# Aedelon/ProteinBERT-PyTorch-Replication

Measured on AMD Instinct MI355X. Metric: sequences/sec (whole node) ProteinBERT pretrain L=512 at 1/2/4/8 MI355X, higher is better.
Workload: dtype bf16; 1 GPU; global_batch=2048, per_gpu_batch=2048, seq_len=512, parallelism=dp1, impl=hip, hip_graph=False

## Files before the change

proteinbert_pytorch_replication_amd/ops/csrc/conv4.hip:

```cpp
#include "mfma.h"

using namespace pbx;
typedef unsigned short bf16_t;

namespace {
constexpr int CH = 128;
constexpr int BM = 128;
constexpr int KS = 9;
constexpr int NI = KS * 8;
constexpr int NPT = BM / 32;


struct FinArgs {
  const bf16_t* dh1;
  const bf16_t* s1;
  const float* st1;
  int T1, BM1;
  const float* sums1;
  int TS1;
  const float* g1;
  float* dgb;
  float eps;
};

template <bool FIN>
__global__ void __launch_bounds__(256, 2) conv_dgrad4_kernel(
    const bf16_t* __restrict__ ds1, const bf16_t* __restrict__ gdn, const bf16_t* __restrict__ gdw,
    const bf16x8* __restrict__ ftn, const bf16x8* __restrict__ ftw, bf16_t* __restrict__ dx,
    bf16_t* __restrict__ dpre_n, bf16_t* __restrict__ dpre_w, int L, int dil, int ilo, int ihi, FinArgs fa) {
  extern __shared__ __attribute__((aligned(16))) unsigned char smem[];
  const int T = (L + BM - 1) / BM;
  int tid0;
  {
    const int n = gridDim.x, orig = blockIdx.x, xcd = orig & 7, qq = n >> 3, rr = n & 7;
    tid0 = (xcd < rr ? xcd * (qq + 1) : rr * (qq + 1) + (xcd - rr) * qq) + (orig >> 3);
  }
  const int b = tid0 / T, t = tid0 - (tid0 / T) * T;
  const int pos0 = t * BM;
  const int half = KS >> 1;
  const int halo_n = half, halo_w = half * dil;
  const int RN = BM + 2 * halo_n;
  unsigned char* an = smem;
  unsigned char* aw = smem + RN * 256;
  const int tid = threadIdx.x, lane = tid & 63, cq = __builtin_amdgcn_readfirstlane(tid >> 6);
  const int r = lane & 31, h = lane >> 5;
  const size_t sbase = (size_t)b * L * CH;
  const ptrdiff_t ibase = ((ptrdiff_t)b * (L + ilo + ihi) + ilo) * CH;
  const __amdgpu_buffer_rsrc_t rn = __builtin_amdgcn_make_buffer_rsrc(
      const_cast<bf16x8*>(ftn + cq * 64), (short)0, (NI * 4 - cq) * 1024, 0x00020000);
  const __amdgpu_buffer_rsrc_t rw = __builtin_amdgcn_make_buffer_rsrc(
      const_cast<bf16x8*>(ftw + cq * 64), (short)0, (NI * 4 - cq) * 1024, 0x00020000);
  auto wfrag = [&](int it) {
    typedef __attribute__((ext_vector_type(4))) unsigned int u32x4;
    const int li = it < NI ? it : it - NI;
    const u32x4 v = __builtin_amdgcn_raw_buffer_load_b128(it < NI ? rn : rw, lane * 16, li * 4096, 0);
    return __builtin_bit_cast(bf16x8, v);
  };
  bf16x8 fr[4];
  fr[0] = wfrag(0);
  fr[1] = wfrag(1);
  fr[2] = wfrag(2);

  uint4 keep[9];
  float csum[8];
  float mean1 = 0.f, rstd1 = 0.f, m1 = 0.f, m2 = 0.f;
  if constexpr (FIN) {
    wave_ln_stats(fa.st1 + (size_t)b * fa.T1 * 2, fa.T1, fa.BM1, L, CH, fa.eps, mean1, rstd1);
    wave_bwd_consts(fa.sums1 + (size_t)b * fa.TS1 * 2, fa.TS1, 1.0f / (float)(L * CH), m1, m2);
#pragma unroll
    for (int e = 0; e < 8; ++e) csum[e] = 0.f;
  }
  auto fin_load = [&](int pos, int c16, uint4& qd, uint4& qs, float4& ga, float4& gb) {
    const int p = min(max(pos, 0), L - 1);
    const size_t off = sbase + (size_t)p * CH + c16 * 8;
    qd = *reinterpret_cast<const uint4*>(fa.dh1 + off);
    qs = *reinterpret_cast<const uint4*>(fa.s1 + off);
    ga = *reinterpret_cast<const float4*>(fa.g1 + (size_t)p * CH + c16 * 8);
    gb = *reinterpret_cast<const float4*>(fa.g1 + (size_t)p * CH + c16 * 8 + 4);
  };
  auto fin_ds1 = [&](bool ok, const uint4& qd, const uint4& qs, const float4& ga, const float4& gb) {
    float dv[8], sv[8], o[8];
    unpack8(qd, dv);
    unpack8(qs, sv);
    const float g[8] = {ga.x, ga.y, ga.z, ga.w, gb.x, gb.y, gb.z, gb.w};
#pragma unroll
    for (int e = 0; e < 8; ++e) o[e] = ok ? rstd1 * (dv[e] * g[e] - m1 - (sv[e] - mean1) * rstd1 * m2) : 0.f;
    return packq8(o);
  };
  auto dpre_of = [&](const uint4& gq, const uint4& pq) {
    float g[8], pv[8], o[8];
    unpack8(gq, g);
    unpack8(pq, pv);
#pragma unroll
    for (int e = 0; e < 8; ++e) o[e] = pv[e] * g[e];
    return packq8(o);
  };
  if constexpr (FIN) {
    const int nchw = (BM + 2 * halo_w) * 16;
    const int joff = halo_w - halo_n;
    for (int base = tid; base < nchw; base += 4 * 256) {
      uint4 qd[4], qs[4], pq[4];
      float4 ga[4], gb[4];
#pragma unroll
      for (int i = 0; i < 4; ++i) {
        const int idx = base + i * 256;
        const int pos = pos0 - halo_w + (idx >> 4);
        fin_load(pos, idx & 15, qd[i], qs[i], ga[i], gb[i]);
        pq[i] = *reinterpret_cast<const uint4*>(gdw + sbase + (size_t)min(max(pos, 0), L - 1) * CH + (idx & 15) * 8);
      }
#pragma unroll
      for (int i = 0; i < 4; ++i) {
        const int idx = base + i * 256;
        if (idx >= nchw) break;
        const int j = idx >> 4, ch = idx & 15;
        const int pos = pos0 - halo_w + j;
        const bool ok = pos >= 0 && pos < L;
        const uint4 dq = fin_ds1(ok, qd[i], qs[i], ga[i], gb[i]);
        const uint4 v = ok ? dpre_of(dq, pq[i]) : make_uint4(0u, 0u, 0u, 0u);
        if (ok && j >= halo_w && j < halo_w + BM)
          *reinterpret_cast<uint4*>(dpre_w + sbase + (size_t)pos * CH + ch * 8) = v;
        *reinterpret_cast<uint4*>(aw + swz256(j, ch)) = v;
        if (j >= joff && j < joff + RN) *reinterpret_cast<uint4*>(an + swz256(j - joff, ch)) = dq;
      }
    }
    __syncthreads();
    const int nch = RN * 16;
#pragma unroll
    for (int mb = 0; mb < 9; mb += 3) {
      uint4 pq[3];
#pragma unroll
      for (int i = 0; i < 3; ++i) {
        const int idx = tid + 256 * (mb + i);
        const int pos = pos0 - halo_n + (idx >> 4);
        pq[i] = *reinterpret_cast<const uint4*>(gdn + sbase + (size_t)min(max(pos, 0), L - 1) * CH + (idx & 15) * 8);
      }
#pragma unroll
      for (int i = 0; i < 3; ++i) {
        const int m = mb + i;
        const int idx = tid + 256 * m;
        const int j = idx >> 4, ch = idx & 15;
        const int pos = pos0 - halo_n + j;
        const bool ok = idx < nch && pos >= 0 && pos < L;
        const uint4 dq = idx < nch ? *reinterpret_cast<const uint4*>(an + swz256(j, ch)) : make_uint4(0u, 0u, 0u, 0u);
        keep[m] = dq;
        if (ok && j >= halo_n && j < halo_n + BM) {
          float t[8];
          unpack8(dq, t);
#pragma unroll
          for (int e = 0; e < 8; ++e) csum[e] += t[e];
        }
        if (idx < nch) {
          const uint4 v = ok ? dpre_of(dq, pq[i]) : make_uint4(0u, 0u, 0u, 0u);
          if (ok && j >= halo_n && j < halo_n + BM)
            *reinterpret_cast<uint4*>(dpre_n + sbase + (size_t)pos * CH + ch * 8) = v;
          *reinterpret_cast<uint4*>(an + swz256(j, ch)) = v;
        }
      }
    }
  }
#pragma unroll 1
  for (int c = 0; c < (FIN ? 0 : 2); ++c) {
    const int halo = c ? halo_w : halo_n;
    const bf16_t* gd = c ? gdw : gdn;
    bf16_t* dpo = c ? dpre_w : dpre_n;
    unsigned char* tile = c ? aw : an;
    const int nch = (BM + 2 * halo) * 16;
    for (int base = tid; base < nch; base += 4 * 256) {
      uint4 gq[4], pq[4];
#pragma unroll
      for (int i = 0; i < 4; ++i) {
        const int idx = base + i * 256;
        const int pos = pos0 - halo + (idx >> 4);
        const bool ok = idx < nch && pos >= -ilo && pos < L + ihi;
        const ptrdiff_t off = ibase + (ptrdiff_t)(ok ? pos : 0) * CH + (idx & 15) * 8;
        gq[i] = ok ? *reinterpret_cast<const uint4*>(ds1 + off) : make_uint4(0u, 0u, 0u, 0u);
        pq[i] = ok ? *reinterpret_cast<const uint4*>(gd + off) : make_uint4(0u, 0u, 0u, 0u);
      }
#pragma unroll
      for (int i = 0; i < 4; ++i) {
        const int idx = base + i * 256;
        if (idx >= nch) break;
        const int j = idx >> 4, ch = idx & 15;
        const int pos = pos0 - halo + j;
        float g[8], pv[8], o[8];
        unpack8(gq[i], g);
        unpack8(pq[i], pv);
#pragma unroll
        for (int e = 0; e < 8; ++e) o[e] = pv[e] * g[e];
        const uint4 v = (pos >= -ilo && pos < L + ihi) ? packq8(o) : make_uint4(0u, 0u, 0u, 0u);
        if (pos >= 0 && pos < L && j >= halo && j < halo + BM)
          *reinterpret_cast<uint4*>(dpo + sbase + (size_t)pos * CH + ch * 8) = v;
        *reinterpret_cast<uint4*>(tile + swz256(j, ch)) = v;
      }
    }
  }
  __syncthreads();

  f32x16_t acc[NPT];
#pragma unroll
  for (int i = 0; i < NPT; ++i) acc[i] = zero16();
  auto rows_of = [&](int c, int k, int& rowb, int& gs) {
    const int rb = (c ? halo_w : halo_n) + r - (k - half) * (c ? dil : 1);
    rowb = rb << 8;
    gs = (h ^ (((rb & 3) << 2) | ((rb >> 2) & 3))) << 4;
  };
  bf16x8 bq[2][NPT];
  int rowb, gs;
  rows_of(0, 0, rowb, gs);
#pragma unroll
  for (int pt = 0; pt < NPT; ++pt) bq[0][pt] = lds_frag(an, (0 ^ gs) + rowb + pt * 8192);
#pragma unroll 1
  for (int c = 0; c < 2; ++c) {
    const unsigned char* as = c ? aw : an;
    for (int k = 0; k < KS; ++k) {
      const int cn = k + 1 < KS ? c : 1, kn = k + 1 < KS ? k + 1 : 0;
      const unsigned char* asn = cn ? aw : an;
      int rowbn, gsn;
      rows_of(cn, kn, rowbn, gsn);
#pragma unroll
      for (int kb = 0; kb < 8; ++kb) {
        const int it = c * NI + k * 8 + kb;
        fr[(kb + 3) & 3] = wfrag(min(it + 3, 2 * NI - 1));
        const unsigned char* nb = kb < 7 ? as : asn;
        const int noff = kb < 7 ? ((32 * (kb + 1)) ^ gs) + rowb : (0 ^ gsn) + rowbn;
#pragma unroll
        for (int pt = 0; pt < NPT; ++pt) bq[(kb + 1) & 1][pt] = lds_frag(nb, noff + pt * 8192);
        __builtin_amdgcn_sched_barrier(0);
#pragma unroll
        for (int pt = 0; pt < NPT; ++pt) acc[pt] = mfma32(fr[kb & 3], bq[kb & 1][pt], acc[pt]);
      }
      rowb = rowbn;
      gs = gsn;
    }
  }

  const int vrows = min(BM, L - pos0);
  float* ft = reinterpret_cast<float*>(smem);
  auto fidx = [&](int p, int c4) { return p * CH + ((c4 ^ (p & 31)) << 2); };
  __syncthreads();
#pragma unroll
  for (int pt = 0; pt < NPT; ++pt)
#pragma unroll
    for (int g = 0; g < 4; ++g) {
      const int c4 = (cq * 32 + 8 * g + 4 * h) >> 2;
      *reinterpret_cast<float4*>(ft + fidx(pt * 32 + r, c4)) =
          make_float4(acc[pt][4 * g], acc[pt][4 * g + 1], acc[pt][4 * g + 2], acc[pt][4 * g + 3]);
    }
  if constexpr (FIN) {
#pragma unroll
    for (int e = 0; e < 8; ++e) {
      csum[e] += __shfl_xor(csum[e], 16, 64);
      csum[e] += __shfl_xor(csum[e], 32, 64);
    }
    float* dsum = ft + BM * CH;
    if (lane < 16) {
#pragma unroll
      for (int e = 0; e < 8; ++e) dsum[cq * CH + lane * 8 + e] = csum[e];
    }
  }
  __syncthreads();
  if constexpr (FIN) {
    if (tid < CH) {
      const float* dsum = ft + BM * CH;
      atomicAdd(fa.dgb + (size_t)b * CH + tid, dsum[tid] + dsum[CH + tid] + dsum[2 * CH + tid] + dsum[3 * CH + tid]);
    }
#pragma unroll
    for (int m = 0; m < 9; ++m) {
      const int row = (tid >> 4) + 16 * m - halo_n, cc = tid & 15;
      if (row < 0 || row >= vrows) continue;
      float gv[8], o[8];
      unpack8(keep[m], gv);
      const float4 f0 = *reinterpret_cast<const float4*>(ft + fidx(row, 2 * cc));
      const float4 f1 = *reinterpret_cast<const float4*>(ft + fidx(row, 2 * cc + 1));
      const float fv[8] = {f0.x, f0.y, f0.z, f0.w, f1.x, f1.y, f1.z, f1.w};
#pragma unroll
      for (int e = 0; e < 8; ++e) o[e] = gv[e] + fv[e];
      *reinterpret_cast<uint4*>(dx + sbase + (size_t)(pos0 + row) * CH + cc * 8) = packq8(o);
    }
    return;
  }
#pragma unroll
  for (int i = 0; i < BM * 16 / 256; ++i) {
    const int idx = tid + 256 * i;
    const int row = idx >> 4, cc = idx & 15;
    if (row >= vrows) continue;
    const size_t off = sbase + (size_t)(pos0 + row) * CH + cc * 8;
    float gv[8], o[8];
    unpack8(*reinterpret_cast<const uint4*>(ds1 + ibase + (ptrdiff_t)(pos0 + row) * CH + cc * 8), gv);
    const float4 f0 = *reinterpret_cast<const float4*>(ft + fidx(row, 2 * cc));
    const float4 f1 = *reinterpret_cast<const float4*>(ft + fidx(row, 2 * cc + 1));
    const float fv[8] = {f0.x, f0.y, f0.z, f0.w, f1.x, f1.y, f1.z, f1.w};
#pragma unroll
    for (int e = 0; e < 8; ++e) o[e] = gv[e] + fv[e];
    *reinterpret_cast<uint4*>(dx + off) = packq8(o);
  }
}

bool dgrad4_attr_set = false;
}

int conv_dgrad4_lds(int dil) {
  const int a = (2 * BM + 8 * (1 + dil)) * 256;
  const int e = BM * CH * 4 + 4 * CH * 4;
  return a > e ? a : e;
}

PBX_EXPORT int pbx_conv_dgrad4x(const void* ds1, const void* gdn, const void* gdw, const void* ftn, const void* ftw,
                                void* dx, void* dpre_n, void* dpre_w, int B, int L, int KS_, int dil, int ilo, int ihi,
                                hipStream_t st) {
  const int lds = conv_dgrad4_lds(dil);
  if (KS_ != KS || dil < 1 || lds > 163840 || B < 1 || L < 1 || ilo < 0 || ihi < 0) return (int)hipErrorInvalidValue;
  if (!dgrad4_attr_set) {
    (void)hipFuncSetAttribute((const void*)conv_dgrad4_kernel<false>, hipFuncAttributeMaxDynamicSharedMemorySize, 163840);
    (void)hipFuncSetAttribute((const void*)conv_dgrad4_kernel<true>, hipFuncAttributeMaxDynamicSharedMemorySize, 163840);
    dgrad4_attr_set = true;
  }
  const int T = (L + BM - 1) / BM;
  hipLaunchKernelGGL(conv_dgrad4_kernel<false>, dim3(B * T), dim3(256), lds, st, (const bf16_t*)ds1,
                     (const bf16_t*)gdn, (const bf16_t*)gdw, (const bf16x8*)ftn, (const bf16x8*)ftw, (bf16_t*)dx,
                     (bf16_t*)dpre_n, (bf16_t*)dpre_w, L, dil, ilo, ihi, FinArgs{});
  return pbx_launch_status();
}

PBX_EXPORT int pbx_conv_dgrad4f(const void* dh1, const void* s1, const float* st1, int T1, int BM1, const float* sums1,
                                int TS1, const float* g1, const void* gdn, const void* gdw, const void* ftn,
                                const void* ftw, void* dx, void* dpre_n, void* dpre_w, float* dgb, int B, int L,
                                int KS_, int dil, float eps, hipStream_t st) {
  const int lds = conv_dgrad4_lds(dil);
  if (KS_ != KS || dil < 1 || lds > 163840 || B < 1 || L < 1 || T1 < 1 || BM1 < 1 || TS1 < 1)
    return (int)hipErrorInvalidValue;
  if (!dgrad4_attr_set) {
    (void)hipFuncSetAttribute((const void*)conv_dgrad4_kernel<false>, hipFuncAttributeMaxDynamicSharedMemorySize, 163840);
    (void)hipFuncSetAttribute((const void*)conv_dgrad4_kernel<true>, hipFuncAttributeMaxDynamicSharedMemorySize, 163840);
    dgrad4_attr_set = true;
  }
  const int T = (L + BM - 1) / BM;
  FinArgs fa{(const bf16_t*)dh1, (const bf16_t*)s1, st1, T1, BM1, sums1, TS1, g1, dgb, eps};
  hipLaunchKernelGGL(conv_dgrad4_kernel<true>, dim3(B * T), dim3(256), lds, st, nullptr, (const bf16_t*)gdn,
                     (const bf16_t*)gdw, (const bf16x8*)ftn, (const bf16x8*)ftw, (bf16_t*)dx, (bf16_t*)dpre_n,
                     (bf16_t*)dpre_w, L, dil, 0, 0, fa);
  return pbx_launch_status();
}
```

proteinbert_pytorch_replication_amd/ops/csrc/mfma.h:

```cpp
#pragma once
#include "common.h"

typedef __attribute__((ext_vector_type(8))) __bf16 bf16x8;
typedef __attribute__((ext_vector_type(4))) short s16x4;

namespace pbx {

__device__ __forceinline__ f32x16_t mfma32(const bf16x8& a, const bf16x8& b, const f32x16_t& c) {
  return __builtin_amdgcn_mfma_f32_32x32x16_bf16(a, b, c, 0, 0, 0);
}

__device__ __forceinline__ f32x16_t zero16() {
  f32x16_t z;
#pragma unroll
  for (int i = 0; i < 16; ++i) z[i] = 0.f;
  return z;
}

__device__ __forceinline__ int swz256(int row, int chunk) {
  return (row << 8) + ((chunk ^ (((row & 3) << 2) | ((row >> 2) & 3))) << 4);
}
__device__ __forceinline__ int swz256e(int row, int col) {
  return swz256(row, col >> 3) + ((col & 7) << 1);
}
__device__ __forceinline__ int swz128(int row, int chunk) {
  return (row << 7) + ((chunk ^ ((row >> 1) & 7)) << 4);
}

__device__ __forceinline__ bf16x8 lds_frag(const unsigned char* base, int byte_off) {
  return *reinterpret_cast<const bf16x8*>(base + byte_off);
}

__device__ __forceinline__ s16x4 lds_tr(const unsigned char* base, int byte_off) {
  typedef __attribute__((address_space(3))) s16x4 lds_s16x4;
  return __builtin_amdgcn_ds_read_tr16_b64_v4i16((lds_s16x4*)(base + byte_off));
}

__device__ __forceinline__ bf16x8 cat_tr(const s16x4& lo, const s16x4& hi) {
  typedef __attribute__((ext_vector_type(8))) short s16x8;
  s16x8 v;
  v[0] = lo[0]; v[1] = lo[1]; v[2] = lo[2]; v[3] = lo[3];
  v[4] = hi[0]; v[5] = hi[1]; v[6] = hi[2]; v[7] = hi[3];
  return __builtin_bit_cast(bf16x8, v);
}

__device__ __forceinline__ int tr_q(int lane) { return (lane >> 2) & 3; }
__device__ __forceinline__ int tr_c(int lane) { return ((lane & 3) << 2) + (((lane >> 4) & 1) << 4); }

__device__ __forceinline__ bf16x8 pack8(const float* v) {
  typedef __attribute__((ext_vector_type(4))) unsigned int u32x4_t;
  u32x4_t u;
#pragma unroll
  for (int i = 0; i < 4; ++i) u[i] = f2bf2(v[2 * i], v[2 * i + 1]);
  return __builtin_bit_cast(bf16x8, u);
}

__device__ __forceinline__ void unpack8(const uint4& q, float* v) {
  v[0] = __uint_as_float(q.x << 16); v[1] = __uint_as_float(q.x & 0xffff0000u);
  v[2] = __uint_as_float(q.y << 16); v[3] = __uint_as_float(q.y & 0xffff0000u);
  v[4] = __uint_as_float(q.z << 16); v[5] = __uint_as_float(q.z & 0xffff0000u);
  v[6] = __uint_as_float(q.w << 16); v[7] = __uint_as_float(q.w & 0xffff0000u);
}
__device__ __forceinline__ void unpack4(const uint2& q, float* v) {
  v[0] = __uint_as_float(q.x << 16); v[1] = __uint_as_float(q.x & 0xffff0000u);
  v[2] = __uint_as_float(q.y << 16); v[3] = __uint_as_float(q.y & 0xffff0000u);
}
__device__ __forceinline__ uint4 packq8(const float* v) {
  uint4 q;
  q.x = f2bf2(v[0], v[1]);
  q.y = f2bf2(v[2], v[3]);
  q.z = f2bf2(v[4], v[5]);
  q.w = f2bf2(v[6], v[7]);
  return q;
}
__device__ __forceinline__ uint2 packq4(const float* v) {
  uint2 q;
  q.x = f2bf2(v[0], v[1]);
  q.y = f2bf2(v[2], v[3]);
  return q;
}
__device__ __forceinline__ float bfround(float f) { return bf2f(f2bf(f)); }

__device__ __forceinline__ float block_sum(float v, float* scratch, int nw) {
  v = wave_reduce_sum(v);
  const int w = threadIdx.x >> 6;
  __syncthreads();
  if ((threadIdx.x & 63) == 0) scratch[w] = v;
  __syncthreads();
  float s = 0.f;
  for (int i = 0; i < nw; ++i) s += scratch[i];
  return s;
}

__device__ __forceinline__ void ln_stats(const float* __restrict__ part, int T, int BM, int L, int C, float eps,
                                         float& mean, float& rstd) {
  float n = 0.f, m = 0.f, M2 = 0.f;
  for (int t = 0; t < T; ++t) {
    const float nt = (float)(min(BM, L - t * BM) * C);
    const float mt = part[2 * t], M2t = part[2 * t + 1];
    const float nn = n + nt;
    const float d = mt - m;
    m += d * (nt / nn);
    M2 += M2t + d * d * (n * nt / nn);
    n = nn;
  }
  mean = m;
  rstd = rsqrtf(M2 / n + eps);
}

__device__ __forceinline__ void ln_bwd_consts(const float* __restrict__ part, int T, float inv_n, float& m1,
                                              float& m2) {
  float a = 0.f, c = 0.f;
  for (int t = 0; t < T; ++t) { a += part[2 * t]; c += part[2 * t + 1]; }
  m1 = a * inv_n;
  m2 = c * inv_n;
}

template <typename SrcF, typename DstF>
__device__ __forceinline__ void stage_chunks(int n, SrcF src, DstF dst) {
  const int bs = blockDim.x;
  for (int base = threadIdx.x; base < n; base += 8 * bs) {
    uint4 v[8];
#pragma unroll
    for (int i = 0; i < 8; ++i) {
      const int idx = base + i * bs;
      v[i] = idx < n ? src(idx) : make_uint4(0u, 0u, 0u, 0u);
    }
#pragma unroll
    for (int i = 0; i < 8; ++i) {
      const int idx = base + i * bs;
      if (idx < n) dst(idx, v[i]);
    }
  }
}

__device__ __forceinline__ void chan_merge(float& n, float& m, float& M2, float nb, float mb, float M2b) {
  const float nn = n + nb;
  if (nn > 0.f) {
    const float d = mb - m;
    const float f = nb / nn;
    m += d * f;
    M2 += M2b + d * d * n * f;
  }
  n = nn;
}

__device__ __forceinline__ void wave_ln_stats(const float* __restrict__ part, int T, int BM, int L, int C, float eps,
                                              float& mean, float& rstd) {
  const int lane = threadIdx.x & 63;
  float n = 0.f, m = 0.f, M2 = 0.f;
  for (int t = lane; t < T; t += 64) {
    const float2 pm = *reinterpret_cast<const float2*>(part + 2 * t);
    chan_merge(n, m, M2, (float)(min(BM, L - t * BM) * C), pm.x, pm.y);
  }
#pragma unroll
  for (int o = 32; o >= 1; o >>= 1) {
    const float nb = __shfl_xor(n, o, 64), mb = __shfl_xor(m, o, 64), M2b = __shfl_xor(M2, o, 64);
    chan_merge(n, m, M2, nb, mb, M2b);
  }
  mean = m;
  rstd = rsqrtf(M2 / n + eps);
}

__device__ __forceinline__ void wave_bwd_consts(const float* __restrict__ part, int T, float inv_n, float& m1,
                                                float& m2) {
  const int lane = threadIdx.x & 63;
  float a = 0.f, c = 0.f;
  for (int t = lane; t < T; t += 64) {
    const float2 pm = *reinterpret_cast<const float2*>(part + 2 * t);
    a += pm.x;
    c += pm.y;
  }
  m1 = wave_reduce_sum(a) * inv_n;
  m2 = wave_reduce_sum(c) * inv_n;
}

__device__ __forceinline__ void wave_chan(float& n, float& m, float& M2) {
#pragma unroll
  for (int o = 32; o >= 1; o >>= 1) {
    const float nb = __shfl_xor(n, o, 64), mb = __shfl_xor(m, o, 64), M2b = __shfl_xor(M2, o, 64);
    chan_merge(n, m, M2, nb, mb, M2b);
  }
}

}
```

Baseline: 108,800 sequences/s.

## Software-pipeline FIN prologue loads with buffer ops and overlap LN stats

```diff
diff --git a/proteinbert_pytorch_replication_amd/ops/csrc/conv4.hip b/proteinbert_pytorch_replication_amd/ops/csrc/conv4.hip
--- a/proteinbert_pytorch_replication_amd/ops/csrc/conv4.hip
+++ b/proteinbert_pytorch_replication_amd/ops/csrc/conv4.hip
@@ -65,19 +65,9 @@
   float csum[8];
   float mean1 = 0.f, rstd1 = 0.f, m1 = 0.f, m2 = 0.f;
   if constexpr (FIN) {
-    wave_ln_stats(fa.st1 + (size_t)b * fa.T1 * 2, fa.T1, fa.BM1, L, CH, fa.eps, mean1, rstd1);
-    wave_bwd_consts(fa.sums1 + (size_t)b * fa.TS1 * 2, fa.TS1, 1.0f / (float)(L * CH), m1, m2);
 #pragma unroll
     for (int e = 0; e < 8; ++e) csum[e] = 0.f;
   }
-  auto fin_load = [&](int pos, int c16, uint4& qd, uint4& qs, float4& ga, float4& gb) {
-    const int p = min(max(pos, 0), L - 1);
-    const size_t off = sbase + (size_t)p * CH + c16 * 8;
-    qd = *reinterpret_cast<const uint4*>(fa.dh1 + off);
-    qs = *reinterpret_cast<const uint4*>(fa.s1 + off);
-    ga = *reinterpret_cast<const float4*>(fa.g1 + (size_t)p * CH + c16 * 8);
-    gb = *reinterpret_cast<const float4*>(fa.g1 + (size_t)p * CH + c16 * 8 + 4);
-  };
   auto fin_ds1 = [&](bool ok, const uint4& qd, const uint4& qs, const float4& ga, const float4& gb) {
     float dv[8], sv[8], o[8];
     unpack8(qd, dv);
@@ -96,66 +86,122 @@
     return packq8(o);
   };
   if constexpr (FIN) {
+    typedef __attribute__((ext_vector_type(4))) unsigned int u32x4;
+    constexpr int VO_DROP = 0x7ffffff0;
+    constexpr int WK = 2;
+    constexpr int NSP = 8;
+    auto issue_fence = [] { asm volatile("" ::: "memory"); };
+    auto rsrc_of = [](const void* p, int bytes) {
+      return __builtin_amdgcn_make_buffer_rsrc(const_cast<void*>(p), (short)0, bytes, 0x00020000);
+    };
+    auto ldq = [](const __amdgpu_buffer_rsrc_t& rs, int vo) {
+      const u32x4 v = __builtin_amdgcn_raw_buffer_load_b128(rs, vo, 0, 0);
+      return make_uint4(v[0], v[1], v[2], v[3]);
+    };
+    auto ldf = [](const __amdgpu_buffer_rsrc_t& rs, int vo) {
+      return __builtin_bit_cast(float4, __builtin_amdgcn_raw_buffer_load_b128(rs, vo, 0, 0));
+    };
+    auto stq = [](const __amdgpu_buffer_rsrc_t& rs, int vo, const uint4& q) {
+      __builtin_amdgcn_raw_buffer_store_b128((u32x4){q.x, q.y, q.z, q.w}, rs, vo, 0, 0);
+    };
+    const int sbytes = L * CH * 2;
+    const __amdgpu_buffer_rsrc_t rdh = rsrc_of(fa.dh1 + sbase, sbytes), rs1 = rsrc_of(fa.s1 + sbase, sbytes);
+    const __amdgpu_buffer_rsrc_t rgw = rsrc_of(gdw + sbase, sbytes), rgn = rsrc_of(gdn + sbase, sbytes);
+    const __amdgpu_buffer_rsrc_t rg1 = rsrc_of(fa.g1, 2 * sbytes);
+    const __amdgpu_buffer_rsrc_t rpw = rsrc_of(dpre_w + sbase, sbytes), rpn = rsrc_of(dpre_n + sbase, sbytes);
     const int nchw = (BM + 2 * halo_w) * 16;
     const int joff = halo_w - halo_n;
-    for (int base = tid; base < nchw; base += 4 * 256) {
-      uint4 qd[4], qs[4], pq[4];
-      float4 ga[4], gb[4];
-#pragma unroll
-      for (int i = 0; i < 4; ++i) {
-        const int idx = base + i * 256;
-        const int pos = pos0 - halo_w + (idx >> 4);
-        fin_load(pos, idx & 15, qd[i], qs[i], ga[i], gb[i]);
-        pq[i] = *reinterpret_cast<const uint4*>(gdw + sbase + (size_t)min(max(pos, 0), L - 1) * CH + (idx & 15) * 8);
-      }
-#pragma unroll
-      for (int i = 0; i < 4; ++i) {
-        const int idx = base + i * 256;
-        if (idx >= nchw) break;
-        const int j = idx >> 4, ch = idx & 15;
+    const int ch = tid & 15;
+    struct WideOps {
+      uint4 qd[WK], qs[WK], pq[WK];
+      float4 ga[WK], gb[WK];
+    };
+    auto wide_load = [&](int trip, WideOps& w) {
+#pragma unroll
+      for (int i = 0; i < WK; ++i) {
+        const int idx = (trip * WK + i) * 256 + tid;
+        const int p = min(max(pos0 - halo_w + (idx >> 4), 0), L - 1);
+        const int vo = (p * CH + ch * 8) * 2;
+        w.qd[i] = ldq(rdh, vo);
+        w.qs[i] = ldq(rs1, vo);
+        w.ga[i] = ldf(rg1, 2 * vo);
+        w.gb[i] = ldf(rg1, 2 * vo + 16);
+        w.pq[i] = ldq(rgw, vo);
+      }
+      issue_fence();
+    };
+    auto wide_conv = [&](int trip, const WideOps& w) {
+#pragma unroll
+      for (int i = 0; i < WK; ++i) {
+        const int idx = (trip * WK + i) * 256 + tid;
+        const int j = idx >> 4;
         const int pos = pos0 - halo_w + j;
         const bool ok = pos >= 0 && pos < L;
-        const uint4 dq = fin_ds1(ok, qd[i], qs[i], ga[i], gb[i]);
-        const uint4 v = ok ? dpre_of(dq, pq[i]) : make_uint4(0u, 0u, 0u, 0u);
-        if (ok && j >= halo_w && j < halo_w + BM)
-          *reinterpret_cast<uint4*>(dpre_w + sbase + (size_t)pos * CH + ch * 8) = v;
-        *reinterpret_cast<uint4*>(aw + swz256(j, ch)) = v;
-        if (j >= joff && j < joff + RN) *reinterpret_cast<uint4*>(an + swz256(j - joff, ch)) = dq;
-      }
-    }
+        uint4 v = make_uint4(0u, 0u, 0u, 0u);
+        if ((trip * WK + i) * 256 + cq * 64 < nchw) {
+          const uint4 dq = fin_ds1(ok, w.qd[i], w.qs[i], w.ga[i], w.gb[i]);
+          v = ok ? dpre_of(dq, w.pq[i]) : make_uint4(0u, 0u, 0u, 0u);
+          *reinterpret_cast<uint4*>(aw + swz256(j, ch)) = v;
+          if (j >= joff && j < joff + RN) *reinterpret_cast<uint4*>(an + swz256(j - joff, ch)) = dq;
+        }
+        stq(rpw, ok && j >= halo_w && j < halo_w + BM ? (pos * CH + ch * 8) * 2 : VO_DROP, v);
+      }
+      issue_fence();
+    };
+    WideOps wa, wb;
+    wide_load(0, wa);
+    const float* st1b = fa.st1 + (size_t)b * fa.T1 * 2;
+    const float* sums1b = fa.sums1 + (size_t)b * fa.TS1 * 2;
+    const float2 pm = ln_part(st1b, lane, fa.T1);
+    float2 ps[NSP];
+#pragma unroll
+    for (int k = 0; k < NSP; ++k) ps[k] = ln_part(sums1b, lane + 64 * k, fa.TS1);
+    issue_fence();
+    uint4 pqn[9];
+#pragma unroll
+    for (int m = 0; m < 9; ++m) {
+      const int p = min(max(pos0 - halo_n + ((tid + 256 * m) >> 4), 0), L - 1);
+      pqn[m] = ldq(rgn, (p * CH + ch * 8) * 2);
+    }
+    issue_fence();
+#pragma unroll
+    for (int i = 0; i < WK; ++i) {
+      __builtin_amdgcn_raw_buffer_store_b32(0u, rpw, VO_DROP - 16 * i, 0, 0);
+      issue_fence();
+    }
+    wave_ln_stats_from(pm, st1b, fa.T1, fa.BM1, L, CH, fa.eps, mean1, rstd1);
+    wave_bwd_consts_from<NSP>(ps, sums1b, fa.TS1, 1.0f / (float)(L * CH), m1, m2);
+    const int ntrip = (nchw + WK * 256 - 1) / (WK * 256);
+    int trip = 0;
+    for (; trip + 2 < ntrip; trip += 2) {
+      wide_load(trip + 1, wb);
+      wide_conv(trip, wa);
+      wide_load(trip + 2, wa);
+      wide_conv(trip + 1, wb);
+    }
+    wide_load(trip + 1, wb);
+    wide_conv(trip, wa);
+    wide_conv(trip + 1, wb);
     __syncthreads();
     const int nch = RN * 16;
 #pragma unroll
-    for (int mb = 0; mb < 9; mb += 3) {
-      uint4 pq[3];
-#pragma unroll
-      for (int i = 0; i < 3; ++i) {
-        const int idx = tid + 256 * (mb + i);
-        const int pos = pos0 - halo_n + (idx >> 4);
-        pq[i] = *reinterpret_cast<const uint4*>(gdn + sbase + (size_t)min(max(pos, 0), L - 1) * CH + (idx & 15) * 8);
-      }
-#pragma unroll
-      for (int i = 0; i < 3; ++i) {
-        const int m = mb + i;
-        const int idx = tid + 256 * m;
-        const int j = idx >> 4, ch = idx & 15;
-        const int pos = pos0 - halo_n + j;
-        const bool ok = idx < nch && pos >= 0 && pos < L;
-        const uint4 dq = idx < nch ? *reinterpret_cast<const uint4*>(an + swz256(j, ch)) : make_uint4(0u, 0u, 0u, 0u);
-        keep[m] = dq;
-        if (ok && j >= halo_n && j < halo_n + BM) {
-          float t[8];
-          unpack8(dq, t);
-#pragma unroll
-          for (int e = 0; e < 8; ++e) csum[e] += t[e];
-        }
-        if (idx < nch) {
-          const uint4 v = ok ? dpre_of(dq, pq[i]) : make_uint4(0u, 0u, 0u, 0u);
-          if (ok && j >= halo_n && j < halo_n + BM)
-            *reinterpret_cast<uint4*>(dpre_n + sbase + (size_t)pos * CH + ch * 8) = v;
-          *reinterpret_cast<uint4*>(an + swz256(j, ch)) = v;
-        }
-      }
+    for (int m = 0; m < 9; ++m) {
+      const int idx = tid + 256 * m;
+      const int j = idx >> 4;
+      const int pos = pos0 - halo_n + j;
+      const bool live = 256 * m + cq * 64 < nch;
+      const bool ok = live && pos >= 0 && pos < L;
+      const bool mid = ok && j >= halo_n && j < halo_n + BM;
+      uint4 dq = make_uint4(0u, 0u, 0u, 0u);
+      if (live) dq = *reinterpret_cast<const uint4*>(an + swz256(j, ch));
+      keep[m] = dq;
+      float t[8];
+      unpack8(dq, t);
+#pragma unroll
+      for (int e = 0; e < 8; ++e) csum[e] += mid ? t[e] : 0.f;
+      const uint4 v = ok ? dpre_of(dq, pqn[m]) : make_uint4(0u, 0u, 0u, 0u);
+      stq(rpn, mid ? (pos * CH + ch * 8) * 2 : VO_DROP, v);
+      if (live) *reinterpret_cast<uint4*>(an + swz256(j, ch)) = v;
     }
   }
 #pragma unroll 1
diff --git a/proteinbert_pytorch_replication_amd/ops/csrc/mfma.h b/proteinbert_pytorch_replication_amd/ops/csrc/mfma.h
--- a/proteinbert_pytorch_replication_amd/ops/csrc/mfma.h
+++ b/proteinbert_pytorch_replication_amd/ops/csrc/mfma.h
@@ -175,12 +175,59 @@
   m2 = wave_reduce_sum(c) * inv_n;
 }
 
-__device__ __forceinline__ void wave_chan(float& n, float& m, float& M2) {
+__device__ __forceinline__ float2 ln_part(const float* __restrict__ part, int t, int T) {
+  return *reinterpret_cast<const float2*>(part + 2 * min(t, T - 1));
+}
+__device__ __forceinline__ float2 ln_part_here(const float* __restrict__ part, int t, int T) {
+  float2 v = ln_part(part, t, T);
+  asm volatile("" : "+v"(v.x), "+v"(v.y));
+  return v;
+}
+__device__ __forceinline__ void wave_ln_stats_from(float2 pm, const float* __restrict__ part, int T, int BM, int L,
+                                                   int C, float eps, float& mean, float& rstd) {
+  const int lane = threadIdx.x & 63;
+  float n = 0.f, m = 0.f, M2 = 0.f;
+  if (lane < T) chan_merge(n, m, M2, (float)(min(BM, L - lane * BM) * C), pm.x, pm.y);
+  for (int t0 = 64; t0 < T; t0 += 64) {
+    const int t = t0 + lane;
+    const float2 pt = ln_part_here(part, t, T);
+    if (t < T) chan_merge(n, m, M2, (float)(min(BM, L - t * BM) * C), pt.x, pt.y);
+  }
 #pragma unroll
   for (int o = 32; o >= 1; o >>= 1) {
     const float nb = __shfl_xor(n, o, 64), mb = __shfl_xor(m, o, 64), M2b = __shfl_xor(M2, o, 64);
     chan_merge(n, m, M2, nb, mb, M2b);
   }
-}
-
-}
+  mean = m;
+  rstd = rsqrtf(M2 / n + eps);
+}
+template <int NP>
+__device__ __forceinline__ void wave_bwd_consts_from(const float2* ps, const float* __restrict__ part, int T,
+                                                     float inv_n, float& m1, float& m2) {
+  const int lane = threadIdx.x & 63;
+  float a = 0.f, c = 0.f;
+#pragma unroll
+  for (int k = 0; k < NP; ++k) {
+    const bool in = lane + 64 * k < T;
+    a = in ? a + ps[k].x : a;
+    c = in ? c + ps[k].y : c;
+  }
+  for (int t0 = 64 * NP; t0 < T; t0 += 64) {
+    const float2 pt = ln_part_here(part, t0 + lane, T);
+    const bool in = t0 + lane < T;
+    a = in ? a + pt.x : a;
+    c = in ? c + pt.y : c;
+  }
+  m1 = wave_reduce_sum(a) * inv_n;
+  m2 = wave_reduce_sum(c) * inv_n;
+}
+
+__device__ __forceinline__ void wave_chan(float& n, float& m, float& M2) {
+#pragma unroll
+  for (int o = 32; o >= 1; o >>= 1) {
+    const float nb = __shfl_xor(n, o, 64), mb = __shfl_xor(m, o, 64), M2b = __shfl_xor(M2, o, 64);
+    chan_merge(n, m, M2, nb, mb, M2b);
+  }
+}
+
+}
```

New measurement: 110,700 sequences/s (median of 6 runs). +1.7%, better.
